# NSAPH-Projects/weather2alert

Measured on AMD Instinct MI355X. Metric: env_steps_per_sec, higher is better.
Workload: dtype f32 tables, fp64 logit accumulation, f32 sigmoid/reward

## Files before the change

### weather2alert_amd/csrc/w2a_step64.hip.h

```cpp
#ifndef W2A_STEP64_HIP_H
#define W2A_STEP64_HIP_H

#ifndef W2A_S64_MIN_ENVS
#define W2A_S64_MIN_ENVS 131072
#endif
#define S64_ENVS 64
#define S64_WAVES (BLOCK / 64)
#define S64_PASS_ENVS 32
#define S64_ROUNDS 4

struct Day {
  uint32_t t, used, streak, hist, ndays, atb, actual, used2, hist2, st_bits, last;
  int32_t budget, act;
  bool done;
};
__device__ __forceinline__ Day derive_day(const u3 h, const u3 c, int32_t act) {
  Day d;
  d.st_bits = 0;
  if (act != 0 && act != 1) { d.st_bits |= W2A_ST_BAD_ACTION; act = 1; }
  d.act = act;
  d.last = D0_LAST(h.a);
  d.t = D0_T(h.a); d.used = D0_USED(h.a); d.streak = D0_STREAK(h.a);
  d.hist = D1_HIST(h.b); d.ndays = D1_NDAYS(h.b);
  d.budget = (int32_t)c.a;
  if (D1_FIN(h.b)) d.st_bits |= W2A_ST_STEP_AFTER_DONE;
  d.atb = ((int32_t)d.used == d.budget) ? 1u : 0u;
  d.actual = (act == 1 && d.atb) ? 0u : (uint32_t)act;
  d.used2 = d.used + d.actual;
  d.hist2 = ((d.hist << 1) | d.actual) & 0x3FFFu;
  d.done = (d.t + 1 >= d.ndays);
  return d;
}
__device__ __forceinline__ float4 runtime_fields(const Day &d, bool fix_lag = false) {
  return make_float4((d.t > 0) ? (float)(fix_lag ? d.last : d.actual) : 0.0f, (float)d.streak,
                     (float)(d.budget - (int32_t)d.used2), (float)__popc(d.hist2));
}
__device__ __forceinline__ void set_comp4(float4 &x, int idx, float v) {
  if (idx == 0) x.x = v;
  if (idx == 1) x.y = v;
  if (idx == 2) x.z = v;
  if (idx == 3) x.w = v;
}

template <bool FIXES>
struct S64WaveT {
  uint2 desc[S64_ENVS];
  float4 rt[S64_ENVS];
  float4 rt2[FIXES ? S64_ENVS : 1];
  float2 z[S64_ENVS];
  float tile[S64_PASS_ENVS * ROWF];
};

#ifndef W2A_S64_SC1
#define W2A_S64_SC1 0
#endif
#ifndef W2A_S64_SKIP_EFF
#define W2A_S64_SKIP_EFF 1
#endif
#ifndef W2A_S64_NT_STATE
#define W2A_S64_NT_STATE 0
#endif
typedef uint32_t v3u __attribute__((ext_vector_type(3)));
__device__ __forceinline__ void st16_sc1(void *p, v4f v) {
  asm volatile("global_store_dwordx4 %0, %1, off sc1" ::"v"(p), "v"(v) : "memory");
}
__device__ __forceinline__ void st12_sc1(void *p, v3u v) {
  asm volatile("global_store_dwordx3 %0, %1, off sc1" ::"v"(p), "v"(v) : "memory");
}
typedef uint32_t v2u __attribute__((ext_vector_type(2)));
__device__ __forceinline__ void st8_sc1(void *p, v2u v) {
  asm volatile("global_store_dwordx2 %0, %1, off sc1" ::"v"(p), "v"(v) : "memory");
}
__device__ __forceinline__ void st4_sc1(void *p, uint32_t v) {
  asm volatile("global_store_dword %0, %1, off sc1" ::"v"(p), "v"(v) : "memory");
}
__device__ __forceinline__ void st1_sc1(void *p, uint32_t v) {
  asm volatile("global_store_byte %0, %1, off sc1" ::"v"(p), "v"(v) : "memory");
}

#ifndef W2A_S64_MIN_WAVES
#define W2A_S64_MIN_WAVES 4
#endif
#ifndef W2A_S64_PRIO
#define W2A_S64_PRIO 3
#endif
#ifndef W2A_S64_TILES
#define W2A_S64_TILES 1
#endif
#ifndef W2A_S64_SERPENTINE
#define W2A_S64_SERPENTINE 1
#endif
__device__ __forceinline__ uint32_t logical_block_rev(uint32_t b, uint32_t per_xcd) {
#if W2A_XCD_SWIZZLE
  return (b & 7u) * per_xcd + (per_xcd - 1u - (b >> 3));
#else
  return 8u * per_xcd - 1u - b;
#endif
}
template <bool WRITE_OBS, bool REWARD_GIVEN, bool PACKED, bool AUTORESET = false, bool FIXES = false, bool NARROW = false>
__device__ __forceinline__ void s64_tile(const StepArgs &a, S64WaveT<FIXES> &sw, const int lane, const int64_t wave_env0,
                                         const bool valid, const uint32_t e, const u3 h, const u3 c, const int32_t act,
                                         const int4 so) {
  const Day d = derive_day(h, c, act);
  const uint32_t t = d.t, used2 = d.used2, hist2 = d.hist2, streak = d.streak, ndays = d.ndays;
  const uint32_t actual = d.actual, atb = d.atb, st_bits = d.st_bits;
  const int32_t budget = d.budget;
  const bool done = d.done;
  const bool restart_in = AUTORESET && a.next_step && D1_FIN(h.b);
  const uint32_t pk0 = NARROW ? pk_rem8(budget - (int32_t)used2) : used2;
  if (NARROW && (uint32_t)budget >= PK_REM_ESCAPE && valid && !restart_in && !(a.skip_finished && D1_FIN(h.b)))
    pk_rem_of(a.st, a.n)[e] = (uint32_t)(budget - (int32_t)used2);
  const uint32_t fx = FIXES ? a.tb.fixes : 0u;
  const bool fix_obs = FIXES && WRITE_OBS && (fx & W2A_FIX_OBS);
  uint32_t need_eff = actual;
  if (a.tb.gate_bits && actual)
    need_eff = (a.tb.gate_bits[t * (uint32_t)a.tb.gate_words + (c.b >> 5)] >> (c.b & 31u)) & 1u;
  {
    const uint32_t day_row = t * (uint32_t)(a.tb.S_w * a.tb.Y) + c.b;
    const uint32_t wrow = NARROW ? c.c : W_COL(c.c) * (uint32_t)a.tb.n_samples + W_SAMPLE(c.c);
    sw.desc[lane] = make_uint2((day_row * (ROWF / 4)) | ((fix_obs && !done) ? 0x80000000u : 0u),
                               (wrow * (2 * ROWF / 4)) | (need_eff << 31));
    sw.rt[lane] = runtime_fields(d, (fx & W2A_FIX_LAG) != 0u);
    if (fix_obs)
      sw.rt2[FIXES ? lane : 0] = make_float4((float)actual, (float)(actual ? streak + 1 : 0), (float)(budget - (int32_t)used2),
                                 (float)__popc(hist2));
  }
  __builtin_amdgcn_fence(__ATOMIC_RELEASE, "wavefront");
  __builtin_amdgcn_wave_barrier();
  __builtin_amdgcn_fence(__ATOMIC_ACQUIRE, "wavefront");

  const int p = lane & 7;
  const int g = lane >> 3;
  const int n_obs = a.tb.n_obs;
  const bool write_me = valid && (!done || fix_obs) && !restart_in;
  const uint32_t next_day = (uint32_t)(a.tb.S_w * a.tb.Y) * (ROWF / 4);
#pragma unroll 1
  for (int pass = 0; pass < S64_ENVS / S64_PASS_ENVS; ++pass) {
    if (REWARD_GIVEN && !WRITE_OBS) break;
    if (wave_env0 + pass * S64_PASS_ENVS >= a.n) break;
    float4 x[S64_ROUNDS], wb[S64_ROUNDS], we[S64_ROUNDS], xo[FIXES ? S64_ROUNDS : 1];
    bool need[S64_ROUNDS], nxt[S64_ROUNDS];
#pragma unroll
    for (int r = 0; r < S64_ROUNDS; ++r) {
      uint2 ds = sw.desc[pass * S64_PASS_ENVS + r * 8 + g];
      need[r] = (ds.y >> 31) != 0u;
      nxt[r] = FIXES && (ds.x >> 31) != 0u;
      if (FIXES) ds.x &= 0x7FFFFFFFu;
      const uint32_t wq = ds.y & 0x7FFFFFFFu;
      x[r] = a.tb.X[ds.x + p];
      if (fix_obs) xo[r] = a.tb.X[ds.x + (nxt[r] ? next_day : 0u) + p];
      wb[r] = we[r] = make_float4(0.f, 0.f, 0.f, 0.f);
      if (!REWARD_GIVEN) {
        wb[r] = a.tb.W[wq + p];
        we[r] = a.tb.W[wq + (need[r] ? ROWF / 4 : 0) + p];
      }
    }
#if W2A_S64_PRIO
    __builtin_amdgcn_s_setprio(W2A_S64_PRIO);
#endif
#pragma unroll
    for (int r = 0; r < S64_ROUNDS; ++r) {
      const int j = pass * S64_PASS_ENVS + r * 8 + g;
      if (p == RT_QUAD) x[r] = sw.rt[j];
      if (FIXES && (fx & W2A_FIX_ALERTS_2WKS) && a.tb.slot_hist2w >= 0) {
        const float a2w = sw.rt[j].w;
        if (p == (a.tb.slot_hist2w >> 2)) set_comp4(x[r], a.tb.slot_hist2w & 3, a2w);
        if (fix_obs && p == (a.tb.slot_hist2w >> 2)) set_comp4(xo[r], a.tb.slot_hist2w & 3, a2w);
      }
      if (fix_obs && p == RT_QUAD) xo[r] = nxt[r] ? sw.rt2[FIXES ? j : 0] : sw.rt[j];
      if (!REWARD_GIVEN) {
      const double x0 = (double)x[r].x, x1 = (double)x[r].y, x2 = (double)x[r].z, x3 = (double)x[r].w;
      double zb = x0 * (double)wb[r].x;
      zb = fma(x1, (double)wb[r].y, zb);
      zb = fma(x2, (double)wb[r].z, zb);
      zb = fma(x3, (double)wb[r].w, zb);
      zb += dpp_f64<0xB1>(zb);
      zb += dpp_f64<0x4E>(zb);
      zb += dpp_f64<0x141>(zb);
      double ze = 0.0;
#if W2A_S64_SKIP_EFF
      if (__any(need[r]))
#endif
      {
        ze = x0 * (double)we[r].x;
        ze = fma(x1, (double)we[r].y, ze);
        ze = fma(x2, (double)we[r].z, ze);
        ze = fma(x3, (double)we[r].w, ze);
        if (p == GATE_QUAD && !(x[r].z > 0.5f)) ze = -__builtin_inf();
        ze += dpp_f64<0xB1>(ze);
        ze += dpp_f64<0x4E>(ze);
        ze += dpp_f64<0x141>(ze);
      }
      if (p == 0) sw.z[j] = make_float2((float)zb, (float)ze);
      }
      if (WRITE_OBS) {
        const int base = (r * 8 + g) * n_obs;
        const int trash = S64_PASS_ENVS * n_obs + (lane & 31);
        const float4 ov = fix_obs ? xo[FIXES ? r : 0] : x[r];
        sw.tile[so.x >= 0 ? base + so.x : trash] = ov.x;
        sw.tile[so.y >= 0 ? base + so.y : trash] = ov.y;
        sw.tile[so.z >= 0 ? base + so.z : trash] = ov.z;
        sw.tile[so.w >= 0 ? base + so.w : trash] = ov.w;
      }
    }
    if (WRITE_OBS) {
      __builtin_amdgcn_fence(__ATOMIC_RELEASE, "wavefront");
      __builtin_amdgcn_wave_barrier();
      __builtin_amdgcn_fence(__ATOMIC_ACQUIRE, "wavefront");
      const int64_t env0 = wave_env0 + pass * S64_PASS_ENVS;
      float *dst = reinterpret_cast<float *>(a.obs) + env0 * n_obs;
      const unsigned long long wm_all = __ballot(write_me);
      const uint32_t wm = (uint32_t)(wm_all >> (pass * S64_PASS_ENVS));
      const bool full = env0 + S64_PASS_ENVS <= a.n;
      if (full && wm == 0xFFFFFFFFu) {
        const int chunks = (S64_PASS_ENVS * n_obs) >> 2;
#pragma unroll
        for (int c0 = 0; c0 < (S64_PASS_ENVS * ROWF) / 4; c0 += 64) {
          const int ch = c0 + lane;
          if (ch < chunks) {
            const v4f v = reinterpret_cast<const v4f *>(sw.tile)[ch];
#if W2A_S64_SC1 & 1
            st16_sc1(reinterpret_cast<v4f *>(dst) + ch, v);
#elif W2A_NT_OBS
            __builtin_nontemporal_store(v, reinterpret_cast<v4f *>(dst) + ch);
#else
            reinterpret_cast<v4f *>(dst)[ch] = v;
#endif
          }
        }
      } else if (wm != 0u) {
        const int total = S64_PASS_ENVS * n_obs;
        for (int i = lane; i < total; i += 64) {
          const int jj = i / n_obs;
          if ((wm >> jj) & 1u) dst[i] = sw.tile[i];
        }
      }
      __builtin_amdgcn_fence(__ATOMIC_RELEASE, "wavefront");
      __builtin_amdgcn_wave_barrier();
      __builtin_amdgcn_fence(__ATOMIC_ACQUIRE, "wavefront");
    }
  }
  if (!WRITE_OBS) {
    __builtin_amdgcn_fence(__ATOMIC_RELEASE, "wavefront");
    __builtin_amdgcn_wave_barrier();
    __builtin_amdgcn_fence(__ATOMIC_ACQUIRE, "wavefront");
  }

#if W2A_S64_PRIO
  __builtin_amdgcn_s_setprio(0);
#endif
  if (AUTORESET && valid && restart_in) {
    a.reward[e] = 0.0f;
    a.done[e] = 0;
  } else if (valid && a.skip_finished && D1_FIN(h.b)) {
    a.reward[e] = 0.0f;
    a.done[e] = 1;
  } else if (valid) {
  float r;
  if (REWARD_GIVEN) {
    r = a.reward[e];
  } else {
    const float2 z = sw.z[lane];
    const float base = sigmoid_f32(z.x);
    const float eff = need_eff ? sigmoid_f32(z.y) : 0.0f;
    r = -(1000.0f / 152.0f) * base * (1.0f - eff);
    if (FIXES && (fx & W2A_FIX_PENALTY) && d.act == 1 && atb) r = -1.0f;
  }
  const uint32_t t2 = done ? t : t + 1;
  const uint32_t streak2 = done ? streak : (actual ? streak + 1 : 0);
  const float ret = __uint_as_float(h.c) + r;
  u3 h2;
  h2.a = pack_d0(t2, used2, streak2, actual, atb);
  h2.b = pack_d1(hist2, ndays, done ? 1u : 0u);
  h2.c = __float_as_uint(ret);
#if W2A_S64_SC1 & 2
  if (PACKED) st8_sc1(&a.st.pk_hot[e], v2u{pk_pack_hot(pk0, streak2, hist2, done ? 1u : 0u), h2.c});
  else st12_sc1(&a.st.hot3[e], v3u{h2.a, h2.b, h2.c});
  if (!REWARD_GIVEN) st4_sc1(&a.reward[e], __float_as_uint(r));
  st1_sc1(&a.done[e], done ? 1u : 0u);
#else
  if (PACKED) a.st.pk_hot[e] = make_uint2(pk_pack_hot(pk0, streak2, hist2, done ? 1u : 0u), h2.c);
  else a.st.hot3[e] = h2;
  if (!REWARD_GIVEN) a.reward[e] = r;
  a.done[e] = done ? 1 : 0;
#endif
  if (PACKED && lane == 0) a.st.pk_day[wave_env0 >> 6] = t2;
  if (done && a.last_return) a.last_return[e] = ret;
  if (st_bits) atomicOr(a.status, (int)st_bits);
  }
  if (AUTORESET) {
    const bool rs = valid && (a.next_step ? restart_in : done);
    const unsigned long long rs_mask = __ballot(rs);
    if (rs_mask) {
      uint2 ds = make_uint2(0xFFFFFFFFu, 0u);
      if (rs) {
        const uint4 cold = load_cold(a.st, e);
        const Episode ep = draw_episode(a.tb, a.rc, (uint64_t)(a.gid0 + e), cold.w + 1, (int32_t)cold.z);
        if (ep.bad) atomicOr(a.status, (int)W2A_ST_BAD_EPISODE);
        store_episode(a.st, e, make_uint4(ep.ep_row, ep.ep_w, (uint32_t)ep.sticky, cold.w + 1),
                      make_uint4(pack_d0(0, 0, 0, 0, 0), pack_d1(0, ep.ndays, 0), __float_as_uint(0.0f), (uint32_t)ep.budget));
        if (PACKED && NARROW) {
          a.st.pk_hot[e] = make_uint2(pk_pack_hot(pk_rem8(ep.budget), 0u, 0u, 0u), __float_as_uint(0.0f));
          reinterpret_cast<uint32_t *>(a.st.pk_c)[e] = pk_narrow_word(ep.ep_row, ep.ep_w, (uint32_t)a.tb.n_samples, a.pk_kw);
          pk_rem_of(a.st, a.n)[e] = (uint32_t)ep.budget;
        } else if (PACKED) {
          a.st.pk_hot[e] = make_uint2(pk_pack_hot(0u, 0u, 0u, 0u), __float_as_uint(0.0f));
          a.st.pk_c[e] = make_uint2(pk_budget16((uint32_t)ep.budget) | (W_COL(ep.ep_w) << 16),
                                    (ep.ep_row & 0x3FFFFFu) | (W_SAMPLE(ep.ep_w) << 22));
        }
        ds = make_uint2(ep.ep_row * (ROWF / 4), (uint32_t)ep.budget);
      }
      if (WRITE_OBS) {
        sw.desc[lane] = ds;
        __builtin_amdgcn_fence(__ATOMIC_RELEASE, "wavefront");
        __builtin_amdgcn_wave_barrier();
        __builtin_amdgcn_fence(__ATOMIC_ACQUIRE, "wavefront");
#pragma unroll 1
        for (int r = 0; r < S64_ENVS / 8; ++r) {
          if (!((rs_mask >> (r * 8)) & 0xFFull)) continue;
          const int j = r * 8 + g;
          const uint2 dj = sw.desc[j];
          if (dj.x != 0xFFFFFFFFu) {
            float4 v = a.tb.X[dj.x + p];
            if (p == RT_QUAD) v = make_float4(0.0f, 0.0f, (float)(int32_t)dj.y, 0.0f);
            if (FIXES && (fx & W2A_FIX_ALERTS_2WKS) && a.tb.slot_hist2w >= 0 && p == (a.tb.slot_hist2w >> 2))
              set_comp4(v, a.tb.slot_hist2w & 3, 0.0f);
            float *row = reinterpret_cast<float *>(a.obs) + (size_t)(wave_env0 + j) * n_obs;
            if (so.x >= 0) row[so.x] = v.x;
            if (so.y >= 0) row[so.y] = v.y;
            if (so.z >= 0) row[so.z] = v.z;
            if (so.w >= 0) row[so.w] = v.w;
          }
        }
      }
      if (PACKED && lane == 0) a.st.pk_day[wave_env0 >> 6] = 0u;
    }
  }
}

template <bool NARROW>
__device__ __forceinline__ void s64_load_packed(const StepArgs &a, uint32_t e, uint32_t day, u3 &h, u3 &c, int32_t &act) {
  if (NARROW) {
    const uint32_t *ew = reinterpret_cast<const uint32_t *>(a.st.pk_c);
#if W2A_S64_NT_STATE & 4
    const v2u phv = __builtin_nontemporal_load(reinterpret_cast<const v2u *>(&a.st.pk_hot[e]));
    const uint2 ph = make_uint2(phv.x, phv.y);
    const uint32_t w = __builtin_nontemporal_load(&ew[e]);
#else
    const uint2 ph = a.st.pk_hot[e];
    const uint32_t w = ew[e];
#endif
    const uint32_t used = 0u;
    c.a = PK_USED(ph.x);
    if (c.a == PK_REM_ESCAPE) c.a = pk_rem_of(a.st, a.n)[e];
    h.a = pack_d0(day, used, PK_STREAK(ph.x), PK_HIST(ph.x) & 1u, 0u);
    h.b = pack_d1(PK_HIST(ph.x), (uint32_t)a.uni_nd, PK_FIN(ph.x));
    h.c = ph.y;
    c.b = w >> a.pk_kw;
    c.c = w & ((1u << a.pk_kw) - 1u);
    act = load_action(a, e);
    return;
  }
#if W2A_S64_NT_STATE & 4
  const v2u phv = __builtin_nontemporal_load(reinterpret_cast<const v2u *>(&a.st.pk_hot[e]));
  const v2u pcv = __builtin_nontemporal_load(reinterpret_cast<const v2u *>(&a.st.pk_c[e]));
  const uint2 ph = make_uint2(phv.x, phv.y), pc = make_uint2(pcv.x, pcv.y);
#else
  const uint2 ph = a.st.pk_hot[e];
  const uint2 pc = a.st.pk_c[e];
#endif
  h.a = pack_d0(day, PK_USED(ph.x), PK_STREAK(ph.x), PK_HIST(ph.x) & 1u, 0u);
  h.b = pack_d1(PK_HIST(ph.x), (uint32_t)a.uni_nd, PK_FIN(ph.x));
  h.c = ph.y;
  c.a = pc.x & 0xFFFFu;
  if (c.a == PK_BUDGET_ESCAPE) c.a = a.st.stepc[e].a;
  c.b = pc.y & 0x3FFFFFu;
  c.c = PACK_W(pc.x >> 16, pc.y >> 22);
  act = load_action(a, e);
}
__device__ __forceinline__ void s64_load_state(const StepArgs &a, uint32_t e, u3 &h, u3 &c, int32_t &act) {
#if W2A_S64_NT_STATE & 1
  const v3u hv = __builtin_nontemporal_load(reinterpret_cast<const v3u *>(&a.st.hot3[e]));
  h.a = hv.x; h.b = hv.y; h.c = hv.z;
#else
  h = a.st.hot3[e];
#endif
#if W2A_S64_NT_STATE & 2
  const v3u cv = __builtin_nontemporal_load(reinterpret_cast<const v3u *>(&a.st.stepc[e]));
  c.a = cv.x; c.b = cv.y; c.c = cv.z;
#else
  c = a.st.stepc[e];
#endif
  act = load_action(a, e);
}

template <bool WRITE_OBS, bool REWARD_GIVEN, bool PACKED = false, bool AUTORESET = false, bool FIXES = false, bool NARROW = false>
__global__ __launch_bounds__(BLOCK, FIXES ? 3 : W2A_S64_MIN_WAVES) void k_step64(const StepArgs a) {
  __shared__ __attribute__((aligned(16))) S64WaveT<FIXES> s_w[S64_WAVES];
  const int tid = threadIdx.x;
  const int lane = tid & 63;
  const int wave = __builtin_amdgcn_readfirstlane(tid >> 6);
  S64WaveT<FIXES> &sw = s_w[wave];
  uint32_t lb = logical_block(blockIdx.x, gridDim.x >> 3);
  int wave_tile = wave;
#if W2A_S64_SERPENTINE
  if (a.walk_rev) {
    lb = logical_block_rev(blockIdx.x, gridDim.x >> 3);
    wave_tile = S64_WAVES - 1 - wave;
  }
#endif
  const int64_t wave_env0 = ((int64_t)lb * S64_WAVES + wave_tile) * (S64_ENVS * W2A_S64_TILES);
  if (wave_env0 >= a.n) return;
  uint32_t dayn = 0;
  if (PACKED) {
    dayn = a.st.pk_day[wave_env0 >> 6];
    if (dayn == W2A_PK_DAY_POISON) {
      if (lane == 0) atomicOr(a.status, (int)W2A_ST_STALE_GRAPH);
      return;
    }
  }
  u3 hn, cn;
  int32_t an;
  {
    const int64_t env = wave_env0 + lane;
    if (PACKED) s64_load_packed<NARROW>(a, (uint32_t)(env < a.n ? env : a.n - 1), dayn, hn, cn, an);
    else s64_load_state(a, (uint32_t)(env < a.n ? env : a.n - 1), hn, cn, an);
  }
  int4 so = make_int4(-1, -1, -1, -1);
  if (WRITE_OBS) so = reinterpret_cast<const int4 *>(a.slot_obs)[lane & 7];
#pragma unroll 1
  for (int i = 0; i < W2A_S64_TILES; ++i) {
    const int64_t env0 = wave_env0 + (int64_t)i * S64_ENVS;
    if (env0 >= a.n) break;
    const int64_t env = env0 + lane;
    const bool valid = env < a.n;
    const uint32_t e = (uint32_t)(valid ? env : (a.n - 1));
    const u3 h = hn, c = cn;
    const int32_t act = an;
    if (i + 1 < W2A_S64_TILES && env0 + S64_ENVS < a.n) {
      const int64_t en = env + S64_ENVS;
      if (PACKED) {
        dayn = a.st.pk_day[(env0 + S64_ENVS) >> 6];
        s64_load_packed<NARROW>(a, (uint32_t)(en < a.n ? en : a.n - 1), dayn == W2A_PK_DAY_POISON ? 0u : dayn, hn, cn, an);
      } else s64_load_state(a, (uint32_t)(en < a.n ? en : a.n - 1), hn, cn, an);
    }
    s64_tile<WRITE_OBS, REWARD_GIVEN, PACKED, AUTORESET, FIXES, PACKED && NARROW>(a, sw, lane, env0, valid, e, h, c, act, so);
    __builtin_amdgcn_fence(__ATOMIC_RELEASE, "wavefront");
    __builtin_amdgcn_wave_barrier();
    __builtin_amdgcn_fence(__ATOMIC_ACQUIRE, "wavefront");
  }
}

__global__ void k_pack_state(StateArrays st, int64_t n, int32_t pk_kw, int32_t n_samples) {
  const int64_t i = (int64_t)blockIdx.x * blockDim.x + threadIdx.x;
  if (i >= n) return;
  const u3 h = st.hot3[i];
  const u3 c = st.stepc[i];
  if (pk_kw >= 0) {
    const int32_t rem = (int32_t)c.a - (int32_t)D0_USED(h.a);
    st.pk_hot[i] = make_uint2(pk_pack_hot(pk_rem8(rem), D0_STREAK(h.a), D1_HIST(h.b), D1_FIN(h.b)), h.c);
    reinterpret_cast<uint32_t *>(st.pk_c)[i] = pk_narrow_word(c.b, c.c, (uint32_t)n_samples, pk_kw);
    pk_rem_of(st, n)[i] = (uint32_t)rem;
  } else {
    st.pk_hot[i] = make_uint2(pk_pack_hot(D0_USED(h.a), D0_STREAK(h.a), D1_HIST(h.b), D1_FIN(h.b)), h.c);
    st.pk_c[i] = make_uint2(pk_budget16(c.a) | (W_COL(c.c) << 16), (c.b & 0x3FFFFFu) | (W_SAMPLE(c.c) << 22));
  }
  if ((i & 63) == 0) st.pk_day[i >> 6] = D0_T(h.a);
}
__global__ void k_unpack_state(StateArrays st, int64_t n, int32_t n_days, int32_t pk_kw) {
  const int64_t i = (int64_t)blockIdx.x * blockDim.x + threadIdx.x;
  if (i >= n) return;
  const uint2 ph = st.pk_hot[i];
  const uint32_t t = st.pk_day[i >> 6];
  const uint32_t hist = PK_HIST(ph.x), fin = PK_FIN(ph.x), last = hist & 1u;
  uint32_t used = PK_USED(ph.x);
  if (pk_kw >= 0) used = (uint32_t)((int32_t)st.stepc[i].a - (int32_t)(used == PK_REM_ESCAPE ? pk_rem_of(st, n)[i] : used));
  const uint32_t atb = ((t > 0 || fin) && (int32_t)(used - last) == (int32_t)st.stepc[i].a) ? 1u : 0u;
  u3 h;
  h.a = pack_d0(t, used, PK_STREAK(ph.x), last, atb);
  h.b = pack_d1(hist, (uint32_t)n_days, fin);
  h.c = ph.y;
  st.hot3[i] = h;
}
__global__ void k_poison_mirror(StateArrays st, int64_t n) {
  const int64_t i = (int64_t)blockIdx.x * blockDim.x + threadIdx.x;
  if (i < ((n + 63) >> 6)) st.pk_day[i] = W2A_PK_DAY_POISON;
}

#endif
```

Before: 31.19 billion.

## Compact effect-logit work into a per-wave list of envs needing it

Builds a per-wave compacted list (via ballot and mbcnt) of envs whose alert effect logit is needed, and computes those fp64 effect dot products only for listed envs in dense rounds. Previously the whole round of effect work ran whenever any lane in it needed it. The baseline loop is also restructured to issue up to 8 rounds per iteration for some template variants, with the first effect batch's loads overlapped with baseline loads. This adds LDS indirection, extra register pressure and an extra tail loop, and gains little when most envs need the effect term.

```diff
diff --git a/weather2alert_amd/csrc/w2a_step64.hip.h b/weather2alert_amd/csrc/w2a_step64.hip.h
--- a/weather2alert_amd/csrc/w2a_step64.hip.h
+++ b/weather2alert_amd/csrc/w2a_step64.hip.h
@@ -8,6 +8,7 @@
 #define S64_WAVES (BLOCK / 64)
 #define S64_PASS_ENVS 32
 #define S64_ROUNDS 4
+#define S64_LIST_ROUNDS 4
 
 struct Day {
   uint32_t t, used, streak, hist, ndays, atb, actual, used2, hist2, st_bits, last;
@@ -48,14 +49,12 @@
   float4 rt[S64_ENVS];
   float4 rt2[FIXES ? S64_ENVS : 1];
   float2 z[S64_ENVS];
+  uint8_t elist[S64_ENVS];
   float tile[S64_PASS_ENVS * ROWF];
 };
 
 #ifndef W2A_S64_SC1
 #define W2A_S64_SC1 0
-#endif
-#ifndef W2A_S64_SKIP_EFF
-#define W2A_S64_SKIP_EFF 1
 #endif
 #ifndef W2A_S64_NT_STATE
 #define W2A_S64_NT_STATE 0
@@ -96,6 +95,10 @@
 #else
   return 8u * per_xcd - 1u - b;
 #endif
+}
+template <bool WRITE_OBS, bool REWARD_GIVEN, bool AUTORESET, bool FIXES>
+__host__ __device__ constexpr int s64_issue_rounds() {
+  return (!WRITE_OBS || (FIXES && !AUTORESET)) ? S64_ROUNDS : 2 * S64_ROUNDS;
 }
 template <bool WRITE_OBS, bool REWARD_GIVEN, bool PACKED, bool AUTORESET = false, bool FIXES = false, bool NARROW = false>
 __device__ __forceinline__ void s64_tile(const StepArgs &a, S64WaveT<FIXES> &sw, const int lane, const int64_t wave_env0,
@@ -115,6 +118,10 @@
   uint32_t need_eff = actual;
   if (a.tb.gate_bits && actual)
     need_eff = (a.tb.gate_bits[t * (uint32_t)a.tb.gate_words + (c.b >> 5)] >> (c.b & 31u)) & 1u;
+  const unsigned long long eff_mask = REWARD_GIVEN ? 0ull : __ballot(need_eff != 0u);
+  const int n_eff = __popcll(eff_mask);
+  if (!REWARD_GIVEN && need_eff)
+    sw.elist[__builtin_amdgcn_mbcnt_hi((uint32_t)(eff_mask >> 32), __builtin_amdgcn_mbcnt_lo((uint32_t)eff_mask, 0u))] = (uint8_t)lane;
   {
     const uint32_t day_row = t * (uint32_t)(a.tb.S_w * a.tb.Y) + c.b;
     const uint32_t wrow = NARROW ? c.c : W_COL(c.c) * (uint32_t)a.tb.n_samples + W_SAMPLE(c.c);
@@ -134,33 +141,54 @@
   const int n_obs = a.tb.n_obs;
   const bool write_me = valid && (!done || fix_obs) && !restart_in;
   const uint32_t next_day = (uint32_t)(a.tb.S_w * a.tb.Y) * (ROWF / 4);
+  constexpr int NI = s64_issue_rounds<WRITE_OBS, REWARD_GIVEN, AUTORESET, FIXES>();
+  auto eff_issue = [&](const int idx, float4 &xe, float4 &we, int &je) {
+    const bool has = idx < n_eff;
+    je = has ? (int)sw.elist[idx & (S64_ENVS - 1)] : g;
+    const uint2 ds = sw.desc[je];
+    xe = a.tb.X[(ds.x & 0x7FFFFFFFu) + p];
+    we = a.tb.W[(ds.y & 0x7FFFFFFFu) + (has ? ROWF / 4 : 0) + p];
+  };
+  auto eff_logit = [&](const int idx, float4 xe, const float4 we, const int je) {
+    if (p == RT_QUAD) xe = sw.rt[je];
+    if (FIXES && (fx & W2A_FIX_ALERTS_2WKS) && a.tb.slot_hist2w >= 0 && p == (a.tb.slot_hist2w >> 2))
+      set_comp4(xe, a.tb.slot_hist2w & 3, sw.rt[je].w);
+    double ze = (double)xe.x * (double)we.x;
+    ze = fma((double)xe.y, (double)we.y, ze);
+    ze = fma((double)xe.z, (double)we.z, ze);
+    ze = fma((double)xe.w, (double)we.w, ze);
+    if (p == GATE_QUAD && !(xe.z > 0.5f)) ze = -__builtin_inf();
+    ze += dpp_f64<0xB1>(ze);
+    ze += dpp_f64<0x4E>(ze);
+    ze += dpp_f64<0x141>(ze);
+    if (p == 0 && idx < n_eff) sw.z[je].y = (float)ze;
+  };
+  float4 lx0 = make_float4(0.f, 0.f, 0.f, 0.f), lw0 = lx0;
+  int lj0 = 0;
+  if (!REWARD_GIVEN && NI < 2 * S64_ROUNDS) eff_issue(g, lx0, lw0, lj0);
 #pragma unroll 1
-  for (int pass = 0; pass < S64_ENVS / S64_PASS_ENVS; ++pass) {
+  for (int r0 = 0; r0 < S64_ENVS / 8; r0 += NI) {
     if (REWARD_GIVEN && !WRITE_OBS) break;
-    if (wave_env0 + pass * S64_PASS_ENVS >= a.n) break;
-    float4 x[S64_ROUNDS], wb[S64_ROUNDS], we[S64_ROUNDS], xo[FIXES ? S64_ROUNDS : 1];
-    bool need[S64_ROUNDS], nxt[S64_ROUNDS];
-#pragma unroll
-    for (int r = 0; r < S64_ROUNDS; ++r) {
-      uint2 ds = sw.desc[pass * S64_PASS_ENVS + r * 8 + g];
-      need[r] = (ds.y >> 31) != 0u;
+    if (wave_env0 + r0 * 8 >= a.n) break;
+    float4 x[NI], wb[NI], xo[FIXES ? NI : 1];
+    bool nxt[NI];
+#pragma unroll
+    for (int r = 0; r < NI; ++r) {
+      uint2 ds = sw.desc[(r0 + r) * 8 + g];
       nxt[r] = FIXES && (ds.x >> 31) != 0u;
       if (FIXES) ds.x &= 0x7FFFFFFFu;
-      const uint32_t wq = ds.y & 0x7FFFFFFFu;
       x[r] = a.tb.X[ds.x + p];
       if (fix_obs) xo[r] = a.tb.X[ds.x + (nxt[r] ? next_day : 0u) + p];
-      wb[r] = we[r] = make_float4(0.f, 0.f, 0.f, 0.f);
-      if (!REWARD_GIVEN) {
-        wb[r] = a.tb.W[wq + p];
-        we[r] = a.tb.W[wq + (need[r] ? ROWF / 4 : 0) + p];
-      }
+      wb[r] = make_float4(0.f, 0.f, 0.f, 0.f);
+      if (!REWARD_GIVEN) wb[r] = a.tb.W[(ds.y & 0x7FFFFFFFu) + p];
+      if (!REWARD_GIVEN && NI == 2 * S64_ROUNDS && r == S64_ROUNDS - 1) eff_issue(g, lx0, lw0, lj0);
     }
 #if W2A_S64_PRIO
     __builtin_amdgcn_s_setprio(W2A_S64_PRIO);
 #endif
 #pragma unroll
-    for (int r = 0; r < S64_ROUNDS; ++r) {
-      const int j = pass * S64_PASS_ENVS + r * 8 + g;
+    for (int r = 0; r < NI; ++r) {
+      const int j = (r0 + r) * 8 + g;
       if (p == RT_QUAD) x[r] = sw.rt[j];
       if (FIXES && (fx & W2A_FIX_ALERTS_2WKS) && a.tb.slot_hist2w >= 0) {
         const float a2w = sw.rt[j].w;
@@ -177,24 +205,19 @@
       zb += dpp_f64<0xB1>(zb);
       zb += dpp_f64<0x4E>(zb);
       zb += dpp_f64<0x141>(zb);
-      double ze = 0.0;
-#if W2A_S64_SKIP_EFF
-      if (__any(need[r]))
-#endif
-      {
-        ze = x0 * (double)we[r].x;
-        ze = fma(x1, (double)we[r].y, ze);
-        ze = fma(x2, (double)we[r].z, ze);
-        ze = fma(x3, (double)we[r].w, ze);
-        if (p == GATE_QUAD && !(x[r].z > 0.5f)) ze = -__builtin_inf();
-        ze += dpp_f64<0xB1>(ze);
-        ze += dpp_f64<0x4E>(ze);
-        ze += dpp_f64<0x141>(ze);
+      if (p == 0) sw.z[j].x = (float)zb;
       }
-      if (p == 0) sw.z[j] = make_float2((float)zb, (float)ze);
-      }
+    }
+    if (!REWARD_GIVEN && r0 == 0) eff_logit(g, lx0, lw0, lj0);
+#pragma unroll
+    for (int half = 0; half < NI / S64_ROUNDS; ++half) {
+    const int e_off = (r0 + half * S64_ROUNDS) * 8;
+    if (half > 0 && wave_env0 + e_off >= a.n) break;
+#pragma unroll
+    for (int rr = 0; rr < S64_ROUNDS; ++rr) {
+      const int r = half * S64_ROUNDS + rr;
       if (WRITE_OBS) {
-        const int base = (r * 8 + g) * n_obs;
+        const int base = (rr * 8 + g) * n_obs;
         const int trash = S64_PASS_ENVS * n_obs + (lane & 31);
         const float4 ov = fix_obs ? xo[FIXES ? r : 0] : x[r];
         sw.tile[so.x >= 0 ? base + so.x : trash] = ov.x;
@@ -207,10 +230,10 @@
       __builtin_amdgcn_fence(__ATOMIC_RELEASE, "wavefront");
       __builtin_amdgcn_wave_barrier();
       __builtin_amdgcn_fence(__ATOMIC_ACQUIRE, "wavefront");
-      const int64_t env0 = wave_env0 + pass * S64_PASS_ENVS;
+      const int64_t env0 = wave_env0 + e_off;
       float *dst = reinterpret_cast<float *>(a.obs) + env0 * n_obs;
       const unsigned long long wm_all = __ballot(write_me);
-      const uint32_t wm = (uint32_t)(wm_all >> (pass * S64_PASS_ENVS));
+      const uint32_t wm = (uint32_t)(wm_all >> e_off);
       const bool full = env0 + S64_PASS_ENVS <= a.n;
       if (full && wm == 0xFFFFFFFFu) {
         const int chunks = (S64_PASS_ENVS * n_obs) >> 2;
@@ -239,12 +262,22 @@
       __builtin_amdgcn_wave_barrier();
       __builtin_amdgcn_fence(__ATOMIC_ACQUIRE, "wavefront");
     }
-  }
-  if (!WRITE_OBS) {
-    __builtin_amdgcn_fence(__ATOMIC_RELEASE, "wavefront");
-    __builtin_amdgcn_wave_barrier();
-    __builtin_amdgcn_fence(__ATOMIC_ACQUIRE, "wavefront");
-  }
+    }
+  }
+  if (!REWARD_GIVEN) {
+#pragma unroll 1
+    for (int k0 = 8; k0 < n_eff; k0 += 8 * S64_LIST_ROUNDS) {
+      float4 lx[S64_LIST_ROUNDS], lw[S64_LIST_ROUNDS];
+      int lj[S64_LIST_ROUNDS];
+#pragma unroll
+      for (int r = 0; r < S64_LIST_ROUNDS; ++r) eff_issue(k0 + r * 8 + g, lx[r], lw[r], lj[r]);
+#pragma unroll
+      for (int r = 0; r < S64_LIST_ROUNDS; ++r) eff_logit(k0 + r * 8 + g, lx[r], lw[r], lj[r]);
+    }
+  }
+  __builtin_amdgcn_fence(__ATOMIC_RELEASE, "wavefront");
+  __builtin_amdgcn_wave_barrier();
+  __builtin_amdgcn_fence(__ATOMIC_ACQUIRE, "wavefront");
 
 #if W2A_S64_PRIO
   __builtin_amdgcn_s_setprio(0);
```

Result: faster. 32.05 billion (median of 6 runs) (+2.8%).
